# Wang-Xiaoyang/resource_packing_self_play

Measured on AMD Instinct MI355X. Metric: self-play episodes/sec (with MCTS node expansions/sec alongside), higher is better.
Workload: dtype f64 PUCT / f32 Q + CNN, u32 bit-board

## Files before the change

### include/rp_engine.h

```cpp
#ifndef RP_ENGINE_H
#define RP_ENGINE_H
#include <stdint.h>
#ifdef __cplusplus
extern "C" {
#endif

#define RP_ABI_VERSION 4

typedef enum rp_status {
    RP_OK = 0,
    RP_ERR_ARG = -1,
    RP_ERR_DEVICE = -2,
    RP_ERR_CAPACITY = -3,
    RP_ERR_ASSERT = -4,
    RP_ERR_STATE = -5
} rp_status;

typedef enum rp_move_rule {
    RP_MOVE_EXTERNAL = 0,
    RP_MOVE_ARGMAX_FIRST = 1,
    RP_MOVE_SAMPLE = 2,
    RP_MOVE_ARGMAX_DRAW = 3
} rp_move_rule;

enum { RP_PHASE_IDLE = 0, RP_PHASE_RUNNING = 1, RP_PHASE_WAIT_EVAL = 2, RP_PHASE_MOVE_READY = 3,
       RP_PHASE_EPISODE_DONE = 4, RP_PHASE_FAILED = 5 };

enum { RP_KIND_WEAK = 0, RP_KIND_F32 = 1, RP_KIND_F64 = 2 };

typedef struct rp_config {
// ... 49 lines not shown
int rp_set_stream(rp_ctx *ctx, void *stream);
int rp_set_step_cap(rp_ctx *ctx, int32_t max_sims_per_step);
int rp_set_compact_rows(rp_ctx *ctx, int32_t enable);
int rp_set_move_rule(rp_ctx *ctx, int32_t move_rule, int32_t onehot_examples);
int rp_set_sims(rp_ctx *ctx, int32_t sims);

int rp_search_step(rp_ctx *ctx, int32_t *n_leaves_out);
int rp_leaf_planes(rp_ctx *ctx, float *planes_dev, int64_t capacity_rows);
int rp_leaf_count_async(rp_ctx *ctx, int32_t *count_host);
int rp_stem_set_weights(rp_ctx *ctx, const float *conv_w_dev, const float *bias_dev);
int rp_leaf_stem(rp_ctx *ctx, float *out_dev, float *out_relu_dev , int64_t capacity_rows,
                 int32_t channels_last );
int rp_nn_pack_conv16(rp_ctx *ctx, const float *w_dev, float *frag_dev);
int rp_nn_value_head(rp_ctx *ctx, const float *z_dev, const float *w_dev, const float *bias_dev, float *out_dev, int64_t B, int32_t K);
int rp_nn_resblock16(rp_ctx *ctx, const float *x_dev, const float *frag0_dev, const float *bias0_dev, const float *frag1_dev, const float *bias1_dev,
                     float *out_dev, float *out_relu_dev , int64_t B, int32_t H, int32_t W);
int rp_nn_resstage16(rp_ctx *ctx, const float *x_dev, const float *frag4_dev, const float *bias4_dev, float *out_dev, float *out_relu_dev, int64_t B,
                     int32_t H, int32_t W);
int rp_nn_pack_conv32(rp_ctx *ctx, const float *w_dev, float *frag_dev, int32_t Cin);
int rp_nn_resstage32(rp_ctx *ctx, const float *x_dev, const float *frag4_dev, const float *bias4_dev, float *out_dev, float *out_relu_dev, int64_t B,
                     int32_t H, int32_t W);
int rp_nn_convpool32(rp_ctx *ctx, const float *x_dev, const float *frag_dev, const float *bias_dev, float *out_dev, int64_t B, int32_t Cin, int32_t H,
                     int32_t W);
int rp_nn_bias_relu(rp_ctx *ctx, float *x_dev, const float *bias_dev, int64_t B, int32_t C, int32_t HW);
int rp_nn_bias_residual(rp_ctx *ctx, const float *x_dev, const float *bias_dev, const float *res_dev, float *out_dev, float *out_relu_dev,
                        int64_t B, int32_t C, int32_t HW);
int rp_nn_bias_pool(rp_ctx *ctx, const float *x_dev, const float *bias_dev, float *out_dev, float *out_relu_dev, int64_t B, int32_t C, int32_t H,
                    int32_t W, int32_t channels_last);
int rp_leaf_states(rp_ctx *ctx, int32_t max_rows, uint64_t *rows_out , uint8_t *remaining_out ,
                   int32_t *slot_out , int32_t *n_out);
int rp_commit_eval(rp_ctx *ctx, const float *pi_dev, const float *v_dev);
int rp_commit_eval_logits(rp_ctx *ctx, const float *logits_dev, const float *v_dev);
int rp_commit_eval_host(rp_ctx *ctx, const float *pi_host, const float *v_host, int32_t n_rows);

int rp_root_counts(rp_ctx *ctx, int32_t first, int32_t count, uint32_t *counts_out);
int rp_game_status(rp_ctx *ctx, int32_t first, int32_t count, int32_t *phase_out, int32_t *sims_done_out,
                   int32_t *moves_out, uint64_t *episode_out);
int rp_last_values(rp_ctx *ctx, int32_t first, int32_t count, double *v_out, int32_t *kind_out);
int rp_advance_roots(rp_ctx *ctx, int32_t first, int32_t count, const int32_t *action, int32_t *ended_out,
                     double *score_out);
int rp_pop_finished(rp_ctx *ctx, int64_t max_n, uint64_t *episode_id_out, int32_t *outcome_out, double *score_out,
                    int32_t *moves_out, int64_t *n_out);
int rp_counters(rp_ctx *ctx, int64_t *out16, int32_t reset);

int rp_examples_count(rp_ctx *ctx, int64_t *n_out);
int rp_examples_tensors(rp_ctx *ctx, int64_t first, int64_t count, float *planes_dev, float *pi_dev, float *value_dev);
// ... 27 lines not shown
```

### resource_packing_self_play_amd/_lib.py

```python
import ctypes as C
import os

import numpy as np

HERE = os.path.dirname(os.path.abspath(__file__))
LIB_PATH = os.environ.get("RP_ENGINE_LIB") or os.path.join(HERE, "csrc", "librp_engine.so")
ABI_VERSION = 4

MOVE_EXTERNAL, MOVE_ARGMAX_FIRST, MOVE_SAMPLE, MOVE_ARGMAX_DRAW = 0, 1, 2, 3
PHASE_IDLE, PHASE_RUNNING, PHASE_WAIT_EVAL, PHASE_MOVE_READY, PHASE_EPISODE_DONE, PHASE_FAILED = range(6)
KIND_WEAK, KIND_F32, KIND_F64 = 0, 1, 2
ERR_ARG, ERR_DEVICE, ERR_CAPACITY, ERR_ASSERT, ERR_STATE = -1, -2, -3, -4, -5
COUNTER_NAMES = ("simulations", "expansions", "terminal_returns", "path_edges", "sum_valid_select", "sum_valid_leaf",
                 "transposition_links", "nodes", "moves", "episodes", "hash_probes", "key_bytes", "sum_visited_select", "visited_new",
                 "reserved0", "reserved1")


class RpConfig(C.Structure):
    _fields_ = [("abi_version", C.c_int32), ("W", C.c_int32), ("H", C.c_int32), ("N", C.c_int32), ("games", C.c_int32),
                ("sims", C.c_int32), ("cpuct", C.c_double), ("alpha", C.c_double), ("node_cap", C.c_int32),
                ("edge_cap", C.c_int32), ("move_rule", C.c_int32), ("auto_restart", C.c_int32), ("reclaim", C.c_int32),
                ("reserved0", C.c_int32), ("seed", C.c_uint64),
                ("tie_salt", C.c_uint64), ("device", C.c_int32), ("vis_cap", C.c_int32), ("stream", C.c_void_p),
                ("max_examples", C.c_int64), ("max_sparse", C.c_int64)]


class EngineError(RuntimeError):
    def __init__(self, code, msg):
        super().__init__("rp_engine error %d: %s" % (code, msg))
        self.code = code
# ... 14 lines not shown
    "rp_begin_pool": (C.c_int, [_vp]),
    "rp_generate_items": (C.c_int, [_vp, _i64, _vp, _i32, _i32, _vp]),
    "rp_set_instance_pool_seeds": (C.c_int, [_vp, _i64, _vp, _i32, _i32, C.c_uint64]),
    "rp_set_instance_meta": (C.c_int, [_vp, _i64, _vp, _vp, _vp]),
    "rp_set_rank_buffer": (C.c_int, [_vp, _vp, _i32]),
    "rp_set_roots": (C.c_int, [_vp, _i32, _i32, _vp, _vp]),
    "rp_set_stream": (C.c_int, [_vp, _vp]),
    "rp_set_step_cap": (C.c_int, [_vp, _i32]),
    "rp_set_compact_rows": (C.c_int, [_vp, _i32]),
    "rp_set_move_rule": (C.c_int, [_vp, _i32, _i32]),
    "rp_set_sims": (C.c_int, [_vp, _i32]),
    "rp_last_values": (C.c_int, [_vp, _i32, _i32, _vp, _vp]),
    "rp_search_step": (C.c_int, [_vp, _vp]),
    "rp_leaf_planes": (C.c_int, [_vp, _vp, _i64]),
    "rp_stem_set_weights": (C.c_int, [_vp, _vp, _vp]),
    "rp_leaf_stem": (C.c_int, [_vp, _vp, _vp, _i64, _i32]),
    "rp_nn_pack_conv16": (C.c_int, [_vp, _vp, _vp]),
    "rp_nn_value_head": (C.c_int, [_vp, _vp, _vp, _vp, _vp, _i64, _i32]),
    "rp_nn_resblock16": (C.c_int, [_vp, _vp, _vp, _vp, _vp, _vp, _vp, _vp, _i64, _i32, _i32]),
    "rp_nn_resstage16": (C.c_int, [_vp, _vp, _vp, _vp, _vp, _vp, _i64, _i32, _i32]),
    "rp_nn_pack_conv32": (C.c_int, [_vp, _vp, _vp, _i32]),
    "rp_nn_convpool32": (C.c_int, [_vp, _vp, _vp, _vp, _vp, _i64, _i32, _i32, _i32]),
    "rp_nn_resstage32": (C.c_int, [_vp, _vp, _vp, _vp, _vp, _vp, _i64, _i32, _i32]),
    "rp_nn_bias_relu": (C.c_int, [_vp, _vp, _vp, _i64, _i32, _i32]),
    "rp_nn_bias_residual": (C.c_int, [_vp, _vp, _vp, _vp, _vp, _vp, _i64, _i32, _i32]),
    "rp_nn_bias_pool": (C.c_int, [_vp, _vp, _vp, _vp, _vp, _i64, _i32, _i32, _i32, _i32]),
    "rp_leaf_states": (C.c_int, [_vp, _i32, _vp, _vp, _vp, _vp]),
    "rp_commit_eval": (C.c_int, [_vp, _vp, _vp]),
    "rp_commit_eval_logits": (C.c_int, [_vp, _vp, _vp]),
    "rp_commit_eval_host": (C.c_int, [_vp, _vp, _vp, _i32]),
    "rp_root_counts": (C.c_int, [_vp, _i32, _i32, _vp]),
    "rp_game_status": (C.c_int, [_vp, _i32, _i32, _vp, _vp, _vp, _vp]),
    "rp_advance_roots": (C.c_int, [_vp, _i32, _i32, _vp, _vp, _vp]),
    "rp_pop_finished": (C.c_int, [_vp, _i64, _vp, _vp, _vp, _vp, _vp]),
    "rp_counters": (C.c_int, [_vp, _vp, _i32]),
    "rp_examples_count": (C.c_int, [_vp, _vp]),
    "rp_examples_tensors": (C.c_int, [_vp, _i64, _i64, _vp, _vp, _vp]),
    "rp_examples_meta": (C.c_int, [_vp, _i64, _i64, _vp, _vp]),
    "rp_examples_clear": (C.c_int, [_vp]),
    "rp_examples_packed_count": (C.c_int, [_vp, _vp, _vp]),
    "rp_examples_packed": (C.c_int, [_vp, _i64, _i64] + [_vp] * 9),
    "rp_expand_examples": (C.c_int, [_vp, _i64, _vp, _i64, _i64] + [_vp] * 10),
    "rp_check": (C.c_int, [_vp]),
    "rp_leaf_count_async": (C.c_int, [_vp, _vp]),
    "rp_tree_size": (C.c_int, [_vp, _i32, _vp, _vp]),
    "rp_arena_peak": (C.c_int, [_vp, _vp, _vp, _vp]),
# ... 242 lines not shown
            raise ValueError("nn_resstage16 needs a channels-last [B, 16, H, W] tensor with H * W <= 640")
        self._timed("k_resstage16 %dx%d" % (H, W), lambda: self._ck(self.L.rp_nn_resstage16(
            self.h, C.c_void_p(x.data_ptr()), C.c_void_p(frag4.data_ptr()), C.c_void_p(bias4.data_ptr()), C.c_void_p(out.data_ptr()),
            C.c_void_p(out_relu.data_ptr()) if out_relu is not None else None, B, H, W)))

    def nn_pack_conv32(self, weight, frag):
        self._ck(self.L.rp_nn_pack_conv32(self.h, C.c_void_p(weight.data_ptr()), C.c_void_p(frag.data_ptr()), int(weight.shape[1])))

    def nn_convpool32(self, x, frag, bias, out):
        B, Cc, H, W = x.shape
        if self._bchw(x)[2] != 1 or self._bchw(out)[2] != 1:
            raise ValueError("nn_convpool32 needs channels-last tensors")
        self._timed("k_convpool32 %d->32 %dx%d" % (Cc, H, W), lambda: self._ck(self.L.rp_nn_convpool32(
            self.h, C.c_void_p(x.data_ptr()), C.c_void_p(frag.data_ptr()), C.c_void_p(bias.data_ptr()), C.c_void_p(out.data_ptr()), B, Cc, H, W)))

    def nn_resstage32(self, x, frag4, bias4, out, out_relu=None):
        B, Cc, H, W = x.shape
        if Cc != 32 or self._bchw(x)[2] != 1 or H * W > 512:
            raise ValueError("nn_resstage32 needs a channels-last [B, 32, H, W] tensor with H * W <= 512")
        self._timed("k_resstage32 %dx%d" % (H, W), lambda: self._ck(self.L.rp_nn_resstage32(
            self.h, C.c_void_p(x.data_ptr()), C.c_void_p(frag4.data_ptr()), C.c_void_p(bias4.data_ptr()), C.c_void_p(out.data_ptr()),
            C.c_void_p(out_relu.data_ptr()) if out_relu is not None else None, B, H, W)))

    def nn_bias_relu(self, x, bias):
        B, Cc, inner = self._bchw(x)
        self._ck(self.L.rp_nn_bias_relu(self.h, C.c_void_p(x.data_ptr()), C.c_void_p(bias.data_ptr()), B, Cc, inner))
        return x

    def nn_bias_residual(self, x, bias, res, out, out_relu=None):
        B, Cc, inner = self._bchw(x)
        self._ck(self.L.rp_nn_bias_residual(self.h, C.c_void_p(x.data_ptr()), C.c_void_p(bias.data_ptr()), C.c_void_p(res.data_ptr()),
                                            C.c_void_p(out.data_ptr()), C.c_void_p(out_relu.data_ptr()) if out_relu is not None else None,
                                            B, Cc, inner))

    def nn_bias_pool(self, x, bias, out, out_relu=None):
        B, Cc, H, W = x.shape
        cl = self._bchw(x)[2] == 1 and H * W > 1
        self._ck(self.L.rp_nn_bias_pool(self.h, C.c_void_p(x.data_ptr()), C.c_void_p(bias.data_ptr()), C.c_void_p(out.data_ptr()),
                                        C.c_void_p(out_relu.data_ptr()) if out_relu is not None else None, B, Cc, H, W, 1 if cl else 0))

    def leaf_count_async(self, pinned_int32, index=0):
        self._ck(self.L.rp_leaf_count_async(self.h, C.c_void_p(pinned_int32.data_ptr() + 4 * int(index))))

    def examples_packed_count(self):
        n, s = _i64(0), _i64(0)
        self._ck(self.L.rp_examples_packed_count(self.h, C.byref(n), C.byref(s)))
# ... 134 lines not shown
```

### resource_packing_self_play_amd/binpacking/pytorch/BinpackingNNet.py

```python
import torch
from torch import nn
from torch.nn import functional as F

STAGE_CHANNELS = (16, 32, 32)
HIDDEN = 256


def _conv3x3(cin, cout):
    return nn.Conv2d(cin, cout, kernel_size=3, padding=1)


class _Residual(nn.Module):
    def __init__(self, ch):
        super().__init__()
        self.conv0 = _conv3x3(ch, ch)
        self.conv1 = _conv3x3(ch, ch)

    def forward(self, x):
        y = self.conv0(F.relu(x))
        y = self.conv1(F.relu(y))
        return y + x


class _Stage(nn.Module):
# ... 27 lines not shown
        cins = (self.in_channels,) + STAGE_CHANNELS[:-1]
        self.conv_seqs = nn.ModuleList(_Stage(ci, co) for ci, co in zip(cins, STAGE_CHANNELS))
        c, h, w = shapes[-1]
        self.hidden_fc = nn.Linear(c * h * w, HIDDEN)
        self.logits_fc = nn.Linear(HIDDEN, self.action_size)
        self.value_fc = nn.Linear(HIDDEN, 1)

    def trunk(self, x):
        for stage in self.conv_seqs:
            x = stage(x)
        x = F.relu(torch.flatten(x, start_dim=1))
        return F.relu(self.hidden_fc(x))

    def heads(self, z):
        return F.log_softmax(self.logits_fc(z), dim=1), torch.tanh(self.value_fc(z))

    def forward(self, x):
        return self.heads(self.trunk(x))

    DENSE_MAX_PIXELS = 9
    STAGE16_MAX_PIXELS = 640
    STAGE32_MAX_PIXELS = 512
    use_resblock_kernel = True
    fused_linear_relu = hasattr(torch, "_addmm_activation")

    def _set_cached(self, key, value):
        if not hasattr(self, "_dense"):
            self._dense = {}
        if key in self._dense and self._dense[key].shape == value.shape:
            self._dense[key].copy_(value)
        else:
            self._dense[key] = value.contiguous()

    def refresh_dense(self):
        shapes = stage_shapes(self.in_channels, self.board_h, self.board_w)
        with torch.no_grad():
            for si, stage in enumerate(self.conv_seqs):
                ch, h, w = shapes[si]
                if h * w > self.DENSE_MAX_PIXELS:
                    continue
                n = ch * h * w
                for bi, blk in enumerate((stage.res_block0, stage.res_block1)):
                    for ci, conv in enumerate((blk.conv0, blk.conv1)):
                        eye = torch.eye(n, device=conv.weight.device, dtype=conv.weight.dtype)
                        key = "%d:b%dc%d" % (si, bi, ci)
                        self._set_cached(key, F.conv2d(eye.view(n, ch, h, w), conv.weight, None, padding=1).flatten(1))
# ... 41 lines not shown
                wt = stage.conv.weight.detach().contiguous()
                keep.append(wt)
                ops.nn_pack_conv32(wt, self._dense[key])
        return keep

    @staticmethod
    def _is_cl(x):
        return x.dim() == 4 and not x.is_contiguous() and x.is_contiguous(memory_format=torch.channels_last)

    def _conv_nobias(self, x, conv, si, which):
        cl = self._is_cl(x)
        mt = getattr(self, "_dense", {}).get("%d:%s%s" % (si, which, ":cl" if cl else ""))
        if mt is None:
            return F.conv2d(x, conv.weight, None, padding=1)
        b, _, h, w = x.shape
        if cl:
            return torch.mm(x.permute(0, 2, 3, 1).reshape(b, -1), mt).view(b, h, w, conv.out_channels).permute(0, 3, 1, 2)
        return torch.mm(x.flatten(1), mt).view(b, conv.out_channels, h, w)

    def forward_from_stem_fused(self, y, y_relu, ops, logits=False):
        cl = self._is_cl(y)
        fmt = torch.channels_last if cl else torch.contiguous_format
        x, xr = y, y_relu
        for si, stage in enumerate(self.conv_seqs):
            ef = getattr(self, "_dense", {}).get("entryfrag:%d" % si) if cl and self.use_resblock_kernel and si > 0 else None
            if ef is not None:
                b, _, h, w = x.shape
                xin, x = x, torch.empty((b, stage.conv.out_channels, (h + 1) // 2, (w + 1) // 2), device=x.device, dtype=x.dtype, memory_format=fmt)
                ops.nn_convpool32(xin, ef, stage.conv.bias, x)
                xr = None
            elif si > 0:
                c = F.conv2d(x, stage.conv.weight, None, padding=1)
                b, ch, h, w = c.shape
                x = torch.empty((b, ch, (h + 1) // 2, (w + 1) // 2), device=c.device, dtype=c.dtype, memory_format=fmt)
                xr = torch.empty_like(x)
                ops.nn_bias_pool(c, stage.conv.bias, x, xr)
            sf = getattr(self, "_dense", {}).get("stagefrag:%d" % si) if cl and self.use_resblock_kernel else None
            if sf is not None:
                last = si == len(self.conv_seqs) - 1
                out = torch.empty_like(x)
                out_r = torch.empty_like(x) if last else None
                (ops.nn_resstage16 if x.shape[1] == 16 else ops.nn_resstage32)(x, sf, self._dense["stagebias:%d" % si], out, out_r)
                x, xr = out, out_r
                continue
            if xr is None:
                xr = torch.relu(x)
            for bi, blk in enumerate((stage.res_block0, stage.res_block1)):
                f0 = getattr(self, "_dense", {}).get("frag:%d:b%dc0" % (si, bi)) if cl and self.use_resblock_kernel and x.shape[1] == 16 else None
                if f0 is not None:
                    out, out_r = torch.empty_like(x), torch.empty_like(x)
                    ops.nn_resblock16(x, f0, blk.conv0.bias, self._dense["frag:%d:b%dc1" % (si, bi)], blk.conv1.bias, out, out_r)
                    x, xr = out, out_r
                    continue
                c0 = self._conv_nobias(xr, blk.conv0, si, "b%dc0" % bi)
                ops.nn_bias_relu(c0, blk.conv0.bias)
                c1 = self._conv_nobias(c0, blk.conv1, si, "b%dc1" % bi)
                out, out_r = torch.empty_like(c1), torch.empty_like(c1)
                ops.nn_bias_residual(c1, blk.conv1.bias, x, out, out_r)
                x, xr = out, out_r
        hw = getattr(self, "_dense", {}).get("hidden:cl") if cl else None
        feats, wmat = (xr.permute(0, 2, 3, 1).reshape(xr.shape[0], -1), hw) if cl and hw is not None else (torch.flatten(xr, start_dim=1), self.hidden_fc.weight)
        if self.fused_linear_relu:
# ... 20 lines not shown
```

### resource_packing_self_play_amd/csrc/rp_engine.hip

```cpp
#include <hip/hip_runtime.h>
#include <math.h>
#include <stdarg.h>
#include <stdint.h>
#include <stdio.h>
#include <stdlib.h>
#include <string.h>

#include <algorithm>
#include <string>
#include <vector>

#include "../../include/rp_engine.h"

#pragma clang fp contract(off)

typedef unsigned long long u64;
typedef unsigned int u32;
typedef unsigned short u16;
typedef unsigned char u8;

#define NONE32 0xFFFFFFFFu
#define NSA_MASK 0x3FFFFFFFu
#define WAVES_PER_BLOCK 4
#define MAX_LEAVES 128
// ... 2298 lines not shown
        }
        RS_T(0)
    }
#undef RS_T
#ifdef RS_STAMP
    if (lane == 0 && out_relu)
        for (int k = 0; k < 10; ++k) atomicAdd((unsigned long long *)out_relu + k, st_acc[k]);
#endif
}

__global__ void k_pack_conv32(const float *w, float *frag, int Cin) {
    const int HQ = Cin / 16;
    int i = blockIdx.x * blockDim.x + threadIdx.x;
    if (i >= 9 * Cin * 32) return;
    const int j = i & 3, l = (i >> 2) & 63, mt = (i >> 8) & 1, h = (i >> 9) % HQ, tap = (i >> 9) / HQ;
    const int co = 16 * mt + (l & 15), ci = (Cin / 4) * (l >> 4) + 4 * h + j;
    frag[i] = w[(co * Cin + ci) * 9 + tap];
}
#define R32_PAD 4
__host__ __device__ constexpr int r32_ps(int cin) { return cin + R32_PAD; }
__host__ __device__ inline int r32_pw(int W) { return W + 1; }
__host__ __device__ inline int r32_imgp(int H, int W) { return (H + 2) * (W + 1) + 1; }
template <int NT, int CIN, int PS, bool TAIL>
__device__ __forceinline__ void r32_conv_t(const float *img, __amdgpu_buffer_rsrc_t frs, int fbase, int fnext, int PW, const int (&abase)[NT], f32x4 (&acc)[NT][2],
                                           f32x4 (&wq)[3][2], int t_abase, int t_voff0, int t_voff1, f32x4 &t_acc, f32x4 (&t_w0)[2], f32x4 (&t_w1)[2]) {
    constexpr int HQ = CIN / 16, NH = 9 * HQ;
    const int voff = lane_id() * 16;
    int z = 0; asm volatile("" : "+v"(z));
    auto a_read = [&](int t, int tap, int h) {
        const int dr = tap / 3, dx = tap - 3 * dr;
        return *(const f32x4 *)(img + abase[t] + z + ((dr * PW + dx) * PS + 4 * h));
    };
    auto at_read = [&](int tap, int h, int w) {
        const int dr = tap / 3, dx = tap - 3 * dr;
        return *(const f32x4 *)(img + t_abase + z + ((dr * PW + dx) * PS + (CIN / 4) * w + 4 * h));
    };
    f32x4 a[NT][HQ], at[HQ][2];
#pragma unroll
    for (int t = 0; t < NT; ++t) {
        acc[t][0] = (f32x4){0.f, 0.f, 0.f, 0.f}; acc[t][1] = (f32x4){0.f, 0.f, 0.f, 0.f};
#pragma unroll
        for (int h = 0; h < HQ; ++h) a[t][h] = a_read(t, 0, h);
    }
    if (TAIL) {
        t_acc = (f32x4){0.f, 0.f, 0.f, 0.f};
#pragma unroll
        for (int h = 0; h < HQ; ++h) { at[h][0] = at_read(0, h, 0); at[h][1] = at_read(0, h, 1); }
    }
#pragma unroll
    for (int s = 0; s < NH; ++s) {
        const int tap = s / HQ, h = s % HQ;
        {
            const int s2 = s + 2, off = s2 < NH ? fbase + s2 * 2048 : fnext + (s2 - NH) * 2048;
            wq[s2 % 3][0] = rs_load_b(frs, voff, off); wq[s2 % 3][1] = rs_load_b(frs, voff, off + 1024);
        }
        const f32x4 w0 = wq[s % 3][0], w1 = wq[s % 3][1];
        __builtin_amdgcn_sched_barrier(0);
#pragma unroll
        for (int j = 0; j < 3; ++j) {
#pragma unroll
            for (int t = 0; t < NT; ++t) {
                acc[t][0] = __builtin_amdgcn_mfma_f32_16x16x4f32(w0[j], a[t][h][j], acc[t][0], 0, 0, 0);
                acc[t][1] = __builtin_amdgcn_mfma_f32_16x16x4f32(w1[j], a[t][h][j], acc[t][1], 0, 0, 0);
            }
            __builtin_amdgcn_sched_barrier(0);
        }
#pragma unroll
        for (int t = 0; t < NT; ++t) {
            acc[t][0] = __builtin_amdgcn_mfma_f32_16x16x4f32(w0[3], a[t][h][3], acc[t][0], 0, 0, 0);
            acc[t][1] = __builtin_amdgcn_mfma_f32_16x16x4f32(w1[3], a[t][h][3], acc[t][1], 0, 0, 0);
            if (tap + 1 < 9) a[t][h] = a_read(t, tap + 1, h);
            __builtin_amdgcn_sched_barrier(0);
        }
        if (TAIL) {
            const f32x4 wa = t_w0[s % 2], wb = t_w1[s % 2];
#pragma unroll
            for (int j = 0; j < 4; ++j) t_acc = __builtin_amdgcn_mfma_f32_4x4x1f32(wa[j], at[h][0][j], t_acc, 0, 0, 0);
#pragma unroll
            for (int j = 0; j < 4; ++j) t_acc = __builtin_amdgcn_mfma_f32_4x4x1f32(wb[j], at[h][1][j], t_acc, 0, 0, 0);
            asm volatile("" : "+v"(t_acc));
            if (tap + 1 < 9) { at[h][0] = at_read(tap + 1, h, 0); at[h][1] = at_read(tap + 1, h, 1); }
            {
                const int s2 = s + 2, off = s2 < NH ? fbase + s2 * 2048 : fnext + (s2 - NH) * 2048;
                t_w0[s % 2] = rs_load_b(frs, t_voff0, off); t_w1[s % 2] = rs_load_b(frs, t_voff1, off);
            }
            __builtin_amdgcn_sched_barrier(0);
        }
    }
}
template <int NT, int CIN, int PS = r32_ps(CIN)>
__device__ __forceinline__ void r32_conv(const float *img, __amdgpu_buffer_rsrc_t frs, int fbase, int fnext, int PW, const int (&abase)[NT], f32x4 (&acc)[NT][2],
                                         f32x4 (&wq)[3][2]) {
    f32x4 d0, d1[2], d2[2];
    r32_conv_t<NT, CIN, PS, false>(img, frs, fbase, fnext, PW, abase, acc, wq, 0, 0, 0, d0, d1, d2);
}
template <int NT>
__global__ void __launch_bounds__(256, 2) k_resstage32(const float *__restrict__ x, const float *__restrict__ frag, const float *__restrict__ bias,
                                                       float *__restrict__ out, float *__restrict__ out_relu, long long B, int S_h, int S_w, int IMGW,
                                                       const int *__restrict__ nrows_dev) {
    constexpr int CIN = 32;
    extern __shared__ __attribute__((aligned(16))) float rb_lds[];
    const int lane = lane_id(), wv = wave_in_block();
    if (nrows_dev) { const long long n = *nrows_dev; if (n < B) B = n; }
    if (((long long)blockIdx.x * 4) * IMGW >= B) return;
    constexpr int PS = r32_ps(CIN);
    const int PW = r32_pw(S_w), PIX = S_h * S_w, IMGP = r32_imgp(S_h, S_w), MP = IMGW * PIX, WAVE_P = IMGW * IMGP + 1;
    int *ptab = (int *)rb_lds;
    float *sbias = rb_lds + 16 * NT;
    float *img = sbias + 128 + (size_t)wv * WAVE_P * PS;
    for (int i = threadIdx.x; i < 16 * NT; i += blockDim.x) {
        int im = i / PIX, pq = i - im * PIX, r = pq / S_w, c = pq - r * S_w;
        ptab[i] = i < MP ? im * IMGP + (r + 1) * PW + c + 1 : 0;
    }
    for (int i = threadIdx.x; i < 128; i += blockDim.x) sbias[i] = bias[i];
    {
        float4 *z4 = (float4 *)img;
        for (int i = lane; i < WAVE_P * PS / 4; i += 64) z4[i] = make_float4(0.f, 0.f, 0.f, 0.f);
    }
    __syncthreads();
    const long long stride_leaves = (long long)gridDim.x * 4 * IMGW;
    long long leaf0 = ((long long)blockIdx.x * 4 + wv) * IMGW;
    if (leaf0 >= B) return;
    const int n = lane & 15, g = lane >> 4;
    int abase[NT], pdst[NT][2];
#pragma unroll
    for (int t = 0; t < NT; ++t) {
        const int m = t * 16 + n, pc = m < MP ? ptab[m] : IMGW * IMGP;
        abase[t] = (ptab[m < MP ? m : 0] - (PW + 1)) * PS + 8 * g;
        pdst[t][0] = pc * PS + 4 * g;
        pdst[t][1] = pc * PS + 16 + 4 * g;
    }
    const __amdgpu_buffer_rsrc_t frs = __builtin_amdgcn_make_buffer_rsrc((void *)frag, 0, 4 * 9 * CIN * 32 * 4, RS_BUF_FLAGS);
    constexpr int CONV_BYTES = 9 * CIN * 32 * 4;
    const int rowoff = n * 128 + g * 16;
    auto task_bytes = [&](long long l0) { return (int)(B - l0 < IMGW ? B - l0 : IMGW) * PIX * 128; };
    f32x4 xv[NT][2], xs[NT][2], wq[3][2];
    auto load_x = [&](long long l0) {
        const __amdgpu_buffer_rsrc_t rs = __builtin_amdgcn_make_buffer_rsrc((void *)(x + (size_t)l0 * PIX * CIN), 0, task_bytes(l0), RS_BUF_FLAGS);
#pragma unroll
        for (int t = 0; t < NT; ++t) { xv[t][0] = rs_load_x(rs, rowoff, t * 2048); xv[t][1] = rs_load_x(rs, rowoff, t * 2048 + 64); }
    };
    auto stage_x = [&]() {
#pragma unroll
        for (int t = 0; t < NT; ++t)
#pragma unroll
            for (int mt = 0; mt < 2; ++mt) { xs[t][mt] = xv[t][mt]; *(f32x4 *)(img + pdst[t][mt]) = rs_relu(xv[t][mt]); }
    };
    load_x(leaf0);
    wq[0][0] = rs_load_b(frs, lane * 16, 0); wq[0][1] = rs_load_b(frs, lane * 16, 1024);
    wq[1][0] = rs_load_b(frs, lane * 16, 2048); wq[1][1] = rs_load_b(frs, lane * 16, 3072);
    stage_x();
    if (leaf0 + stride_leaves < B) load_x(leaf0 + stride_leaves);
    for (; leaf0 < B; leaf0 += stride_leaves) {
        const int nbytes = task_bytes(leaf0);
        const __amdgpu_buffer_rsrc_t ors = __builtin_amdgcn_make_buffer_rsrc((void *)(out + (size_t)leaf0 * PIX * CIN), 0, nbytes, RS_BUF_FLAGS);
        f32x4 acc[NT][2];
// ... 3 lines not shown
        {
            R32_BIAS(0);
#pragma unroll
            for (int t = 0; t < NT; ++t) { *(f32x4 *)(img + pdst[t][0]) = rs_relu(acc[t][0] + ba); *(f32x4 *)(img + pdst[t][1]) = rs_relu(acc[t][1] + bb); }
        }
        lds_sync();
        r32_conv<NT, CIN>(img, frs, CONV_BYTES, 2 * CONV_BYTES, PW, abase, acc, wq);
        {
            R32_BIAS(1);
#pragma unroll
            for (int t = 0; t < NT; ++t) {
                xs[t][0] = (acc[t][0] + ba) + xs[t][0]; xs[t][1] = (acc[t][1] + bb) + xs[t][1];
                *(f32x4 *)(img + pdst[t][0]) = rs_relu(xs[t][0]); *(f32x4 *)(img + pdst[t][1]) = rs_relu(xs[t][1]);
            }
        }
        lds_sync();
        r32_conv<NT, CIN>(img, frs, 2 * CONV_BYTES, 3 * CONV_BYTES, PW, abase, acc, wq);
        {
            R32_BIAS(2);
#pragma unroll
            for (int t = 0; t < NT; ++t) { *(f32x4 *)(img + pdst[t][0]) = rs_relu(acc[t][0] + ba); *(f32x4 *)(img + pdst[t][1]) = rs_relu(acc[t][1] + bb); }
        }
        lds_sync();
        r32_conv<NT, CIN>(img, frs, 3 * CONV_BYTES, 0, PW, abase, acc, wq);
        {
            R32_BIAS(3);
#pragma unroll
            for (int t = 0; t < NT; ++t) {
                acc[t][0] = (acc[t][0] + ba) + xs[t][0]; acc[t][1] = (acc[t][1] + bb) + xs[t][1];
                __builtin_amdgcn_raw_buffer_store_b128(__builtin_bit_cast(u32x4, acc[t][0]), ors, rowoff, t * 2048, RS_STREAM_AUX);
                __builtin_amdgcn_raw_buffer_store_b128(__builtin_bit_cast(u32x4, acc[t][1]), ors, rowoff, t * 2048 + 64, RS_STREAM_AUX);
            }
        }
#undef R32_BIAS
        if (out_relu != nullptr) {
            const __amdgpu_buffer_rsrc_t rrs = __builtin_amdgcn_make_buffer_rsrc((void *)(out_relu + (size_t)leaf0 * PIX * CIN), 0, nbytes, RS_BUF_FLAGS);
#pragma unroll
            for (int t = 0; t < NT; ++t) {
                __builtin_amdgcn_raw_buffer_store_b128(__builtin_bit_cast(u32x4, rs_relu(acc[t][0])), rrs, rowoff, t * 2048, RS_STREAM_AUX);
                __builtin_amdgcn_raw_buffer_store_b128(__builtin_bit_cast(u32x4, rs_relu(acc[t][1])), rrs, rowoff, t * 2048 + 64, RS_STREAM_AUX);
            }
        }
        if (leaf0 + stride_leaves < B) {
            stage_x();
            if (leaf0 + 2 * stride_leaves < B) load_x(leaf0 + 2 * stride_leaves);
        }
    }
}

#define CP_PS 36
#ifdef CP_STAMP
__device__ unsigned long long g_cp_stamp[8];
#endif
template <int NT, int CIN, bool TAIL = false>
__global__ void __launch_bounds__(256, 2) k_convpool32(const float *__restrict__ x, const float *__restrict__ frag, const float *__restrict__ bias,
                                                       float *__restrict__ out, long long B, int S_h, int S_w, int IMGW, int wave_floats,
                                                       const int *__restrict__ nrows_dev) {
    constexpr int XQ = CIN / 16;
// ... 65 lines not shown
    wq[0][0] = rs_load_b(frs, lane * 16, 0); wq[0][1] = rs_load_b(frs, lane * 16, 1024);
    wq[1][0] = rs_load_b(frs, lane * 16, 2048); wq[1][1] = rs_load_b(frs, lane * 16, 3072);
    if (TAIL) {
        t_w0[0] = rs_load_b(frs, t_voff0, 0); t_w1[0] = rs_load_b(frs, t_voff1, 0);
        t_w0[1] = rs_load_b(frs, t_voff0, 2048); t_w1[1] = rs_load_b(frs, t_voff1, 2048);
    }
#ifdef CP_STAMP
    unsigned long long st_acc[8] = {0, 0, 0, 0, 0, 0, 0, 0}, st_last = __builtin_amdgcn_s_memtime();
#define CP_T(k) { unsigned long long now_ = __builtin_amdgcn_s_memtime(); st_acc[k] += now_ - st_last; st_last = now_; }
#else
#define CP_T(k)
#endif
    for (; leaf0 < B; leaf0 += stride_leaves) {
        const int nimg = (int)(B - leaf0 < IMGW ? B - leaf0 : IMGW);
#pragma unroll
        for (int t = 0; t < NT; ++t)
#pragma unroll
            for (int q = 0; q < XQ; ++q) *(f32x4 *)(img + pin[t] + 16 * q) = xv[t][q];
        if (TAIL) *(f32x4 *)(img + pin_t) = xvt;
        if (leaf0 + stride_leaves < B) load_x(leaf0 + stride_leaves);
        f32x4 acc[NT][2];
        lds_sync();
        CP_T(0)
        r32_conv_t<NT, CIN, PS, TAIL>(img, frs, 0, 0, PW, abase, acc, wq, t_abase, t_voff0, t_voff1, t_acc, t_w0, t_w1);
        CP_T(1)
        lds_sync();
#pragma unroll
        for (int t = 0; t < NT; ++t) {
            *(f32x4 *)(img + pin[t]) = acc[t][0] + ba;
            *(f32x4 *)(img + pin[t] + 16) = acc[t][1] + bb;
        }
        if (TAIL) {
            f32x4 r;
#pragma unroll
            for (int k = 0; k < 4; ++k) {
                const float b0 = __shfl(ba[k], 16 * (cg & 3)), b1 = __shfl(bb[k], 16 * (cg & 3));
                r[k] = (t_acc[k] + __shfl_xor(t_acc[k], 4)) + (cg < 4 ? b0 : b1);
            }
            if (kk == 0) *(f32x4 *)(img + pout_t) = r;
        }
        lds_sync();
        CP_T(2)
        float4 *o4 = (float4 *)(out + (size_t)leaf0 * PP * 32);
        for (int pq = lane >> 3; pq < nimg * PP; pq += 8) {
            const int info = pool[pq], ctr = info & 0xFFFF;
            const int up = (info >> 16) & 1, down = (info >> 17) & 1, left = (info >> 18) & 1, right = (info >> 19) & 1;
            const float4 *row = (const float4 *)(img + ctr * PS) + cq;
// ... 1063 lines not shown
            RSW_LAUNCH(2, 4) RSW_LAUNCH(3, 4) RSW_LAUNCH(4, 4) RSW_LAUNCH(3, 8) RSW_LAUNCH(4, 8)
            default: return fail(ctx, RP_ERR_ARG, "rp_nn_resstage32: unsupported image size");
        }
#undef RSW_LAUNCH
        HIPCHK(ctx, hipGetLastError());
        return RP_OK;
    }
    const size_t img_pixels = (size_t)r32_imgp(H, W);
    auto lds_bytes = [&](int k) { return ((size_t)16 * ((k * PIX + 15) / 16) + 128 + 4 * (k * img_pixels + 1) * r32_ps(32)) * sizeof(float); };
    int imgw_max = 80 / PIX;
    while (imgw_max > 1 && lds_bytes(imgw_max) > 78 * 1024) --imgw_max;
    const int imgw = pick_leaves_per_wave(B, PIX, imgw_max);
    const int nt = (imgw * PIX + 15) / 16;
    const size_t lds = lds_bytes(imgw);
    if (lds > ctx->lds_per_cu) return fail(ctx, RP_ERR_ARG, "rp_nn_resstage32: a %dx%d image needs %zu bytes of LDS per workgroup, the device has %zu per CU", H, W, lds, ctx->lds_per_cu);
    const long long tasks = (B + imgw - 1) / imgw;
    static const int rs32_wgs = getenv("RP_STAGE32_WGS") ? atoi(getenv("RP_STAGE32_WGS")) : 2;
    const int per_cu = (int)std::max<size_t>(1, std::min<size_t>((size_t)rs32_wgs, ctx->lds_per_cu / lds));
    const dim3 grid((unsigned)std::min<long long>((tasks + 3) / 4, (long long)ctx->n_cu * per_cu)), block(256);
#define RS_LAUNCH(NT_)                                                                                                                              \
    case NT_:                                                                                                                                       \
        { const int rc_ = allow_lds(ctx, (const void *)k_resstage32<NT_>, lds, "rp_nn_resstage32"); if (rc_ != RP_OK) return rc_; }                \
        hipLaunchKernelGGL(k_resstage32<NT_>, grid, block, lds, ctx->stream, x_dev, frag4_dev, bias4_dev, out_dev, out_relu_dev,                    \
                           (long long)B, (int)H, (int)W, imgw, ctx->nn_rows_dev);                                                                   \
        break;
    switch (nt) {
        RS_LAUNCH(1) RS_LAUNCH(2) RS_LAUNCH(3) RS_LAUNCH(4) RS_LAUNCH(5)
        default: return fail(ctx, RP_ERR_ARG, "rp_nn_resstage32: unsupported image size");
    }
#undef RS_LAUNCH
    HIPCHK(ctx, hipGetLastError());
    return RP_OK;
}

extern "C" int rp_leaf_states(rp_ctx *ctx, int32_t max_rows, uint64_t *rows_out, uint8_t *remaining_out, int32_t *slot_out, int32_t *n_out) {
    if (!ctx || max_rows < 0 || !rows_out || !remaining_out || !slot_out || !n_out) return fail(ctx, RP_ERR_ARG, "rp_leaf_states: bad argument");
    const DP &d = ctx->d;
    if (d.rows_identity) return fail(ctx, RP_ERR_STATE, "rp_leaf_states: call rp_search_step with n_leaves_out first (compact rows)");
    int n = 0;
    HIPCHK(ctx, hipMemcpyAsync(&n, d.eval_count, sizeof(int), hipMemcpyDeviceToHost, ctx->stream));
    HIPCHK(ctx, hipStreamSynchronize(ctx->stream));
    n = std::min(n, (int)max_rows);
    *n_out = n;
    if (n == 0) return RP_OK;
    Scratch s(ctx);
    u64 *drows = s.up((const u64 *)nullptr, (size_t)n * d.H); NEED(drows);
    u8 *drem = s.up((const u8 *)nullptr, (size_t)n * d.N); NEED(drem);
    int *dslot = s.up((const int *)nullptr, (size_t)n); NEED(dslot);
    DISPATCH(ctx, k_leaf_states, grid_for(n), d, drows, drem, dslot, n);
    HIPCHK(ctx, hipMemcpyAsync(rows_out, drows, (size_t)n * d.H * 8, hipMemcpyDeviceToHost, ctx->stream));
    HIPCHK(ctx, hipMemcpyAsync(remaining_out, drem, (size_t)n * d.N, hipMemcpyDeviceToHost, ctx->stream));
    HIPCHK(ctx, hipMemcpyAsync(slot_out, dslot, (size_t)n * sizeof(int), hipMemcpyDeviceToHost, ctx->stream));
    HIPCHK(ctx, hipStreamSynchronize(ctx->stream));
// ... 459 lines not shown
```

Measured before the change: 1395.

## Fuse 32-channel residual stage with next stage's entry conv and max-pool

Adds a POOL variant of k_resstage32 that, after the stage's final residual add, runs the next stage's entry 3x3 conv and 3x3 stride-2 max-pool out of LDS, writing only the pooled output. It prefetches the entry-conv weights through a second buffer resource in the conv pipeline. The Python forward uses this fused path by default whenever consecutive 32-channel stages fit the LDS plan. This removes a full-resolution activation write and read plus one kernel launch per stage boundary. In exchange LDS use rises and per-workgroup work grows, which may lower occupancy.

```diff
diff --git a/include/rp_engine.h b/include/rp_engine.h
--- a/include/rp_engine.h
+++ b/include/rp_engine.h
@@ -5,7 +5,7 @@
 extern "C" {
 #endif
 
-#define RP_ABI_VERSION 4
+#define RP_ABI_VERSION 5
 
 typedef enum rp_status {
     RP_OK = 0,
@@ -101,6 +101,9 @@
                      int32_t H, int32_t W);
 int rp_nn_convpool32(rp_ctx *ctx, const float *x_dev, const float *frag_dev, const float *bias_dev, float *out_dev, int64_t B, int32_t Cin, int32_t H,
                      int32_t W);
+int rp_nn_stage_fusable(rp_ctx *ctx, int32_t C, int64_t B, int32_t H, int32_t W);
+int rp_nn_resstage32_convpool(rp_ctx *ctx, const float *x_dev, const float *frag4_dev, const float *bias4_dev, const float *entry_frag_dev,
+                              const float *entry_bias_dev, float *out_pooled_dev, int64_t B, int32_t H, int32_t W);
 int rp_nn_bias_relu(rp_ctx *ctx, float *x_dev, const float *bias_dev, int64_t B, int32_t C, int32_t HW);
 int rp_nn_bias_residual(rp_ctx *ctx, const float *x_dev, const float *bias_dev, const float *res_dev, float *out_dev, float *out_relu_dev,
                         int64_t B, int32_t C, int32_t HW);
diff --git a/resource_packing_self_play_amd/_lib.py b/resource_packing_self_play_amd/_lib.py
--- a/resource_packing_self_play_amd/_lib.py
+++ b/resource_packing_self_play_amd/_lib.py
@@ -5,7 +5,7 @@
 
 HERE = os.path.dirname(os.path.abspath(__file__))
 LIB_PATH = os.environ.get("RP_ENGINE_LIB") or os.path.join(HERE, "csrc", "librp_engine.so")
-ABI_VERSION = 4
+ABI_VERSION = 5
 
 MOVE_EXTERNAL, MOVE_ARGMAX_FIRST, MOVE_SAMPLE, MOVE_ARGMAX_DRAW = 0, 1, 2, 3
 PHASE_IDLE, PHASE_RUNNING, PHASE_WAIT_EVAL, PHASE_MOVE_READY, PHASE_EPISODE_DONE, PHASE_FAILED = range(6)
@@ -66,6 +66,8 @@
     "rp_nn_pack_conv32": (C.c_int, [_vp, _vp, _vp, _i32]),
     "rp_nn_convpool32": (C.c_int, [_vp, _vp, _vp, _vp, _vp, _i64, _i32, _i32, _i32]),
     "rp_nn_resstage32": (C.c_int, [_vp, _vp, _vp, _vp, _vp, _vp, _i64, _i32, _i32]),
+    "rp_nn_stage_fusable": (C.c_int, [_vp, _i32, _i64, _i32, _i32]),
+    "rp_nn_resstage32_convpool": (C.c_int, [_vp, _vp, _vp, _vp, _vp, _vp, _vp, _i64, _i32, _i32]),
     "rp_nn_bias_relu": (C.c_int, [_vp, _vp, _vp, _i64, _i32, _i32]),
     "rp_nn_bias_residual": (C.c_int, [_vp, _vp, _vp, _vp, _vp, _vp, _i64, _i32, _i32]),
     "rp_nn_bias_pool": (C.c_int, [_vp, _vp, _vp, _vp, _vp, _i64, _i32, _i32, _i32, _i32]),
@@ -354,6 +356,21 @@
             self.h, C.c_void_p(x.data_ptr()), C.c_void_p(frag4.data_ptr()), C.c_void_p(bias4.data_ptr()), C.c_void_p(out.data_ptr()),
             C.c_void_p(out_relu.data_ptr()) if out_relu is not None else None, B, H, W)))
 
+    def nn_stage_fusable(self, x):
+        B, Cc, H, W = x.shape
+        rc = self.L.rp_nn_stage_fusable(self.h, Cc, B, H, W)
+        if rc < 0:
+            self._ck(rc)
+        return rc == 1
+
+    def nn_resstage32_convpool(self, x, frag4, bias4, entry_frag, entry_bias, out_pooled):
+        B, Cc, H, W = x.shape
+        if Cc != 32 or self._bchw(x)[2] != 1 or self._bchw(out_pooled)[2] != 1 or tuple(out_pooled.shape) != (B, 32, (H + 1) // 2, (W + 1) // 2):
+            raise ValueError("nn_resstage32_convpool needs channels-last [B, 32, H, W] -> [B, 32, (H+1)//2, (W+1)//2] tensors")
+        self._timed("k_resstage32+convpool32 %dx%d" % (H, W), lambda: self._ck(self.L.rp_nn_resstage32_convpool(
+            self.h, C.c_void_p(x.data_ptr()), C.c_void_p(frag4.data_ptr()), C.c_void_p(bias4.data_ptr()), C.c_void_p(entry_frag.data_ptr()),
+            C.c_void_p(entry_bias.data_ptr()), C.c_void_p(out_pooled.data_ptr()), B, H, W)))
+
     def nn_bias_relu(self, x, bias):
         B, Cc, inner = self._bchw(x)
         self._ck(self.L.rp_nn_bias_relu(self.h, C.c_void_p(x.data_ptr()), C.c_void_p(bias.data_ptr()), B, Cc, inner))
diff --git a/resource_packing_self_play_amd/binpacking/pytorch/BinpackingNNet.py b/resource_packing_self_play_amd/binpacking/pytorch/BinpackingNNet.py
--- a/resource_packing_self_play_amd/binpacking/pytorch/BinpackingNNet.py
+++ b/resource_packing_self_play_amd/binpacking/pytorch/BinpackingNNet.py
@@ -1,3 +1,5 @@
+import os
+
 import torch
 from torch import nn
 from torch.nn import functional as F
@@ -73,6 +75,7 @@
     STAGE16_MAX_PIXELS = 640
     STAGE32_MAX_PIXELS = 512
     use_resblock_kernel = True
+    use_stage_fusion = os.environ.get("RP_STAGE_FUSE", "1") != "0"
     fused_linear_relu = hasattr(torch, "_addmm_activation")
 
     def _set_cached(self, key, value):
@@ -160,9 +163,12 @@
         cl = self._is_cl(y)
         fmt = torch.channels_last if cl else torch.contiguous_format
         x, xr = y, y_relu
+        entered = False
         for si, stage in enumerate(self.conv_seqs):
             ef = getattr(self, "_dense", {}).get("entryfrag:%d" % si) if cl and self.use_resblock_kernel and si > 0 else None
-            if ef is not None:
+            if entered:
+                entered = False
+            elif ef is not None:
                 b, _, h, w = x.shape
                 xin, x = x, torch.empty((b, stage.conv.out_channels, (h + 1) // 2, (w + 1) // 2), device=x.device, dtype=x.dtype, memory_format=fmt)
                 ops.nn_convpool32(xin, ef, stage.conv.bias, x)
@@ -176,6 +182,14 @@
             sf = getattr(self, "_dense", {}).get("stagefrag:%d" % si) if cl and self.use_resblock_kernel else None
             if sf is not None:
                 last = si == len(self.conv_seqs) - 1
+                nf = None if last or not self.use_stage_fusion else self._dense.get("entryfrag:%d" % (si + 1))
+                if nf is not None and hasattr(ops, "nn_stage_fusable") and ops.nn_stage_fusable(x):
+                    b, _, h, w = x.shape
+                    nxt = self.conv_seqs[si + 1].conv
+                    out = torch.empty((b, nxt.out_channels, (h + 1) // 2, (w + 1) // 2), device=x.device, dtype=x.dtype, memory_format=fmt)
+                    ops.nn_resstage32_convpool(x, sf, self._dense["stagebias:%d" % si], nf, nxt.bias, out)
+                    x, xr, entered = out, None, True
+                    continue
                 out = torch.empty_like(x)
                 out_r = torch.empty_like(x) if last else None
                 (ops.nn_resstage16 if x.shape[1] == 16 else ops.nn_resstage32)(x, sf, self._dense["stagebias:%d" % si], out, out_r)
diff --git a/resource_packing_self_play_amd/csrc/rp_engine.hip b/resource_packing_self_play_amd/csrc/rp_engine.hip
--- a/resource_packing_self_play_amd/csrc/rp_engine.hip
+++ b/resource_packing_self_play_amd/csrc/rp_engine.hip
@@ -2344,8 +2344,8 @@
 __host__ __device__ inline int r32_pw(int W) { return W + 1; }
 __host__ __device__ inline int r32_imgp(int H, int W) { return (H + 2) * (W + 1) + 1; }
 template <int NT, int CIN, int PS, bool TAIL>
-__device__ __forceinline__ void r32_conv_t(const float *img, __amdgpu_buffer_rsrc_t frs, int fbase, int fnext, int PW, const int (&abase)[NT], f32x4 (&acc)[NT][2],
-                                           f32x4 (&wq)[3][2], int t_abase, int t_voff0, int t_voff1, f32x4 &t_acc, f32x4 (&t_w0)[2], f32x4 (&t_w1)[2]) {
+__device__ __forceinline__ void r32_conv_t(const float *img, __amdgpu_buffer_rsrc_t frs, __amdgpu_buffer_rsrc_t nrs, int fbase, int fnext, int PW,
+                                           const int (&abase)[NT], f32x4 (&acc)[NT][2], f32x4 (&wq)[3][2], int t_abase, int t_voff0, int t_voff1, f32x4 &t_acc, f32x4 (&t_w0)[2], f32x4 (&t_w1)[2]) {
     constexpr int HQ = CIN / 16, NH = 9 * HQ;
     const int voff = lane_id() * 16;
     int z = 0; asm volatile("" : "+v"(z));
@@ -2374,7 +2374,8 @@
         const int tap = s / HQ, h = s % HQ;
         {
             const int s2 = s + 2, off = s2 < NH ? fbase + s2 * 2048 : fnext + (s2 - NH) * 2048;
-            wq[s2 % 3][0] = rs_load_b(frs, voff, off); wq[s2 % 3][1] = rs_load_b(frs, voff, off + 1024);
+            const __amdgpu_buffer_rsrc_t rs2 = s2 < NH ? frs : nrs;
+            wq[s2 % 3][0] = rs_load_b(rs2, voff, off); wq[s2 % 3][1] = rs_load_b(rs2, voff, off + 1024);
         }
         const f32x4 w0 = wq[s % 3][0], w1 = wq[s % 3][1];
         __builtin_amdgcn_sched_barrier(0);
@@ -2404,7 +2405,8 @@
             if (tap + 1 < 9) { at[h][0] = at_read(tap + 1, h, 0); at[h][1] = at_read(tap + 1, h, 1); }
             {
                 const int s2 = s + 2, off = s2 < NH ? fbase + s2 * 2048 : fnext + (s2 - NH) * 2048;
-                t_w0[s % 2] = rs_load_b(frs, t_voff0, off); t_w1[s % 2] = rs_load_b(frs, t_voff1, off);
+                const __amdgpu_buffer_rsrc_t rs2 = s2 < NH ? frs : nrs;
+                t_w0[s % 2] = rs_load_b(rs2, t_voff0, off); t_w1[s % 2] = rs_load_b(rs2, t_voff1, off);
             }
             __builtin_amdgcn_sched_barrier(0);
         }
@@ -2414,27 +2416,43 @@
 __device__ __forceinline__ void r32_conv(const float *img, __amdgpu_buffer_rsrc_t frs, int fbase, int fnext, int PW, const int (&abase)[NT], f32x4 (&acc)[NT][2],
                                          f32x4 (&wq)[3][2]) {
     f32x4 d0, d1[2], d2[2];
-    r32_conv_t<NT, CIN, PS, false>(img, frs, fbase, fnext, PW, abase, acc, wq, 0, 0, 0, d0, d1, d2);
-}
-template <int NT>
+    r32_conv_t<NT, CIN, PS, false>(img, frs, frs, fbase, fnext, PW, abase, acc, wq, 0, 0, 0, d0, d1, d2);
+}
+template <int NT, int CIN, int PS = r32_ps(CIN)>
+__device__ __forceinline__ void r32_conv_x(const float *img, __amdgpu_buffer_rsrc_t frs, __amdgpu_buffer_rsrc_t nrs, int fbase, int fnext, int PW,
+                                           const int (&abase)[NT], f32x4 (&acc)[NT][2], f32x4 (&wq)[3][2]) {
+    f32x4 d0, d1[2], d2[2];
+    r32_conv_t<NT, CIN, PS, false>(img, frs, nrs, fbase, fnext, PW, abase, acc, wq, 0, 0, 0, d0, d1, d2);
+}
+template <int NT, bool POOL = false>
 __global__ void __launch_bounds__(256, 2) k_resstage32(const float *__restrict__ x, const float *__restrict__ frag, const float *__restrict__ bias,
                                                        float *__restrict__ out, float *__restrict__ out_relu, long long B, int S_h, int S_w, int IMGW,
-                                                       const int *__restrict__ nrows_dev) {
+                                                       const int *__restrict__ nrows_dev, const float *__restrict__ efrag = nullptr,
+                                                       const float *__restrict__ ebias = nullptr, float *__restrict__ pooled = nullptr) {
     constexpr int CIN = 32;
     extern __shared__ __attribute__((aligned(16))) float rb_lds[];
     const int lane = lane_id(), wv = wave_in_block();
     if (nrows_dev) { const long long n = *nrows_dev; if (n < B) B = n; }
     if (((long long)blockIdx.x * 4) * IMGW >= B) return;
-    constexpr int PS = r32_ps(CIN);
+    constexpr int PS = r32_ps(CIN), NBIAS = POOL ? 160 : 128;
     const int PW = r32_pw(S_w), PIX = S_h * S_w, IMGP = r32_imgp(S_h, S_w), MP = IMGW * PIX, WAVE_P = IMGW * IMGP + 1;
+    const int Hp = (S_h + 1) >> 1, Wp = (S_w + 1) >> 1, PP = Hp * Wp;
     int *ptab = (int *)rb_lds;
     float *sbias = rb_lds + 16 * NT;
-    float *img = sbias + 128 + (size_t)wv * WAVE_P * PS;
+    int *pool = (int *)(sbias + NBIAS);
+    float *img = sbias + NBIAS + (POOL ? (IMGW * PP + 3) & ~3 : 0) + (size_t)wv * WAVE_P * PS;
     for (int i = threadIdx.x; i < 16 * NT; i += blockDim.x) {
         int im = i / PIX, pq = i - im * PIX, r = pq / S_w, c = pq - r * S_w;
         ptab[i] = i < MP ? im * IMGP + (r + 1) * PW + c + 1 : 0;
     }
     for (int i = threadIdx.x; i < 128; i += blockDim.x) sbias[i] = bias[i];
+    if (POOL) {
+        for (int i = threadIdx.x; i < 32; i += blockDim.x) sbias[128 + i] = ebias[i];
+        for (int i = threadIdx.x; i < IMGW * PP; i += blockDim.x) {
+            int im = i / PP, pp = i - im * PP, pr = pp / Wp, px = pp - pr * Wp;
+            pool[i] = (im * IMGP + (2 * pr + 1) * PW + 2 * px + 1) | ((pr > 0) << 16) | ((2 * pr + 1 < S_h) << 17) | ((px > 0) << 18) | ((2 * px + 1 < S_w) << 19);
+        }
+    }
     {
         float4 *z4 = (float4 *)img;
         for (int i = lane; i < WAVE_P * PS / 4; i += 64) z4[i] = make_float4(0.f, 0.f, 0.f, 0.f);
@@ -2454,6 +2472,8 @@
     }
     const __amdgpu_buffer_rsrc_t frs = __builtin_amdgcn_make_buffer_rsrc((void *)frag, 0, 4 * 9 * CIN * 32 * 4, RS_BUF_FLAGS);
     constexpr int CONV_BYTES = 9 * CIN * 32 * 4;
+    const __amdgpu_buffer_rsrc_t efrs = POOL ? __builtin_amdgcn_make_buffer_rsrc((void *)efrag, 0, CONV_BYTES, RS_BUF_FLAGS) : frs;
+    const int cq = lane & 7;
     const int rowoff = n * 128 + g * 16;
     auto task_bytes = [&](long long l0) { return (int)(B - l0 < IMGW ? B - l0 : IMGW) * PIX * 128; };
     f32x4 xv[NT][2], xs[NT][2], wq[3][2];
@@ -2503,8 +2523,42 @@
             for (int t = 0; t < NT; ++t) { *(f32x4 *)(img + pdst[t][0]) = rs_relu(acc[t][0] + ba); *(f32x4 *)(img + pdst[t][1]) = rs_relu(acc[t][1] + bb); }
         }
         lds_sync();
-        r32_conv<NT, CIN>(img, frs, 3 * CONV_BYTES, 0, PW, abase, acc, wq);
-        {
+        r32_conv_x<NT, CIN>(img, frs, efrs, 3 * CONV_BYTES, 0, PW, abase, acc, wq);
+        if (POOL) {
+            {
+                R32_BIAS(3);
+#pragma unroll
+                for (int t = 0; t < NT; ++t) {
+                    *(f32x4 *)(img + pdst[t][0]) = (acc[t][0] + ba) + xs[t][0]; *(f32x4 *)(img + pdst[t][1]) = (acc[t][1] + bb) + xs[t][1];
+                }
+            }
+            lds_sync();
+            r32_conv_x<NT, CIN>(img, efrs, frs, 0, 0, PW, abase, acc, wq);
+            {
+                R32_BIAS(4);
+#pragma unroll
+                for (int t = 0; t < NT; ++t) { *(f32x4 *)(img + pdst[t][0]) = acc[t][0] + ba; *(f32x4 *)(img + pdst[t][1]) = acc[t][1] + bb; }
+            }
+            lds_sync();
+            const int nimg = (int)(B - leaf0 < IMGW ? B - leaf0 : IMGW);
+            float4 *o4 = (float4 *)(pooled + (size_t)leaf0 * PP * 32);
+            for (int pq = lane >> 3; pq < nimg * PP; pq += 8) {
+                const int info = pool[pq], ctr = info & 0xFFFF;
+                const int up = (info >> 16) & 1, down = (info >> 17) & 1, left = (info >> 18) & 1, right = (info >> 19) & 1;
+                const float4 *row = (const float4 *)(img + ctr * PS) + cq;
+                const int ou = up ? -PW : 0, od = down ? PW : 0, ol = left ? -1 : 0, orr = right ? 1 : 0;
+                constexpr int Q = PS / 4;
+                const float4 v0 = row[0], v1 = row[ol * Q], v2 = row[orr * Q], v3 = row[ou * Q], v4 = row[(ou + ol) * Q], v5 = row[(ou + orr) * Q],
+                             v6 = row[od * Q], v7 = row[(od + ol) * Q], v8 = row[(od + orr) * Q];
+                float4 m;
+                m.x = fmaxf(fmaxf(fmaxf(v0.x, v1.x), fmaxf(v2.x, v3.x)), fmaxf(fmaxf(v4.x, v5.x), fmaxf(fmaxf(v6.x, v7.x), v8.x)));
+                m.y = fmaxf(fmaxf(fmaxf(v0.y, v1.y), fmaxf(v2.y, v3.y)), fmaxf(fmaxf(v4.y, v5.y), fmaxf(fmaxf(v6.y, v7.y), v8.y)));
+                m.z = fmaxf(fmaxf(fmaxf(v0.z, v1.z), fmaxf(v2.z, v3.z)), fmaxf(fmaxf(v4.z, v5.z), fmaxf(fmaxf(v6.z, v7.z), v8.z)));
+                m.w = fmaxf(fmaxf(fmaxf(v0.w, v1.w), fmaxf(v2.w, v3.w)), fmaxf(fmaxf(v4.w, v5.w), fmaxf(fmaxf(v6.w, v7.w), v8.w)));
+                o4[pq * 8 + cq] = m;
+            }
+            lds_sync();
+        } else {
             R32_BIAS(3);
 #pragma unroll
             for (int t = 0; t < NT; ++t) {
@@ -2514,7 +2568,7 @@
             }
         }
 #undef R32_BIAS
-        if (out_relu != nullptr) {
+        if (!POOL && out_relu != nullptr) {
             const __amdgpu_buffer_rsrc_t rrs = __builtin_amdgcn_make_buffer_rsrc((void *)(out_relu + (size_t)leaf0 * PIX * CIN), 0, nbytes, RS_BUF_FLAGS);
 #pragma unroll
             for (int t = 0; t < NT; ++t) {
@@ -2626,7 +2680,7 @@
         f32x4 acc[NT][2];
         lds_sync();
         CP_T(0)
-        r32_conv_t<NT, CIN, PS, TAIL>(img, frs, 0, 0, PW, abase, acc, wq, t_abase, t_voff0, t_voff1, t_acc, t_w0, t_w1);
+        r32_conv_t<NT, CIN, PS, TAIL>(img, frs, frs, 0, 0, PW, abase, acc, wq, t_abase, t_voff0, t_voff1, t_acc, t_w0, t_w1);
         CP_T(1)
         lds_sync();
 #pragma unroll
@@ -3736,13 +3790,65 @@
     case NT_:                                                                                                                                       \
         { const int rc_ = allow_lds(ctx, (const void *)k_resstage32<NT_>, lds, "rp_nn_resstage32"); if (rc_ != RP_OK) return rc_; }                \
         hipLaunchKernelGGL(k_resstage32<NT_>, grid, block, lds, ctx->stream, x_dev, frag4_dev, bias4_dev, out_dev, out_relu_dev,                    \
-                           (long long)B, (int)H, (int)W, imgw, ctx->nn_rows_dev);                                                                   \
+                           (long long)B, (int)H, (int)W, imgw, ctx->nn_rows_dev, (const float *)nullptr, (const float *)nullptr, (float *)nullptr); \
         break;
     switch (nt) {
         RS_LAUNCH(1) RS_LAUNCH(2) RS_LAUNCH(3) RS_LAUNCH(4) RS_LAUNCH(5)
         default: return fail(ctx, RP_ERR_ARG, "rp_nn_resstage32: unsupported image size");
     }
 #undef RS_LAUNCH
+    HIPCHK(ctx, hipGetLastError());
+    return RP_OK;
+}
+
+struct Fuse32Plan { int imgw, nt; size_t lds; };
+static bool fuse32_plan(const rp_ctx *ctx, long long B, int H, int W, Fuse32Plan *pl) {
+    static const int enabled = getenv("RP_STAGE32_FUSE") ? atoi(getenv("RP_STAGE32_FUSE")) : 1;
+    const int PIX = H * W;
+    if (!enabled || H < 1 || W < 1 || PIX > 80 || B < 1) return false;
+    const size_t img_pixels = (size_t)r32_imgp(H, W);
+    const int PPn = ((H + 1) / 2) * ((W + 1) / 2);
+    auto lds_bytes = [&](int k) {
+        return ((size_t)16 * ((k * PIX + 15) / 16) + 160 + (((size_t)k * PPn + 3) & ~(size_t)3) + 4 * (k * img_pixels + 1) * r32_ps(32)) * sizeof(float);
+    };
+    int imgw_max = 80 / PIX;
+    while (imgw_max > 1 && lds_bytes(imgw_max) > 78 * 1024) --imgw_max;
+    pl->imgw = pick_leaves_per_wave(B, PIX, imgw_max);
+    pl->nt = (pl->imgw * PIX + 15) / 16;
+    pl->lds = lds_bytes(pl->imgw);
+    return pl->nt <= 5 && pl->lds <= ctx->lds_per_cu;
+}
+
+extern "C" int rp_nn_stage_fusable(rp_ctx *ctx, int32_t C, int64_t B, int32_t H, int32_t W) {
+    if (!ctx || B < 0 || H < 1 || W < 1) return fail(ctx, RP_ERR_ARG, "rp_nn_stage_fusable: bad argument");
+    Fuse32Plan pl;
+    return C == 32 && (B == 0 || fuse32_plan(ctx, B, H, W, &pl)) ? 1 : 0;
+}
+
+extern "C" int rp_nn_resstage32_convpool(rp_ctx *ctx, const float *x_dev, const float *frag4_dev, const float *bias4_dev, const float *entry_frag_dev,
+                                         const float *entry_bias_dev, float *out_pooled_dev, int64_t B, int32_t H, int32_t W) {
+    if (!ctx || !x_dev || !frag4_dev || !bias4_dev || !entry_frag_dev || !entry_bias_dev || !out_pooled_dev || B < 0 || H < 1 || W < 1)
+        return fail(ctx, RP_ERR_ARG, "rp_nn_resstage32_convpool: bad argument");
+    if (B == 0) return RP_OK;
+    Fuse32Plan pl;
+    if (!fuse32_plan(ctx, B, H, W, &pl))
+        return fail(ctx, RP_ERR_ARG, "rp_nn_resstage32_convpool: %dx%d images are not fused (rp_nn_stage_fusable); use rp_nn_resstage32 + rp_nn_convpool32", H, W);
+    const int imgw = pl.imgw;
+    const size_t lds = pl.lds;
+    const long long tasks = (B + imgw - 1) / imgw;
+    const int per_cu = (int)std::max<size_t>(1, std::min<size_t>(2, ctx->lds_per_cu / lds));
+    const dim3 grid((unsigned)std::min<long long>((tasks + 3) / 4, (long long)ctx->n_cu * per_cu)), block(256);
+#define RSF_LAUNCH(NT_)                                                                                                                             \
+    case NT_:                                                                                                                                       \
+        { const int rc_ = allow_lds(ctx, (const void *)k_resstage32<NT_, true>, lds, "rp_nn_resstage32_convpool"); if (rc_ != RP_OK) return rc_; } \
+        hipLaunchKernelGGL((k_resstage32<NT_, true>), grid, block, lds, ctx->stream, x_dev, frag4_dev, bias4_dev, (float *)nullptr, (float *)nullptr, \
+                           (long long)B, (int)H, (int)W, imgw, ctx->nn_rows_dev, entry_frag_dev, entry_bias_dev, out_pooled_dev);                   \
+        break;
+    switch (pl.nt) {
+        RSF_LAUNCH(1) RSF_LAUNCH(2) RSF_LAUNCH(3) RSF_LAUNCH(4) RSF_LAUNCH(5)
+        default: return fail(ctx, RP_ERR_ARG, "rp_nn_resstage32_convpool: unsupported image size");
+    }
+#undef RSF_LAUNCH
     HIPCHK(ctx, hipGetLastError());
     return RP_OK;
 }
```

Result: no change. 1405 (median of 6 runs) (+0.7%).
